# AbnerVictor/OOD-GAN-inversion

Hardware: AMD Instinct MI355X
Metric: 1024² face inversions/sec (100 W+ steps) (higher is better)
Workload: dtype f16-split (hi+lo f16 operands, f32 accumulate): 3 MFMA/product in every forward conv (fp32-equivalent), 2 in the input-gradient convs (back-propagated gradient rounded to f16 before each contraction, weights keep hi+lo); dL/dW+ vs the float64 reference 1.4e-5..3.6e-5 ('f16s': 1.3e-5..2.6e-5, the ref

## Files before the change

ood-gan-inversion_amd/csrc/conv_f16s_t2big.hip:

```cpp
#include "conv_common.hpp"
#include "sform.hpp"
#include <cstdint>
#include <cstdlib>
#include <type_traits>

using namespace oodgan;

typedef _Float16 half8 __attribute__((ext_vector_type(8)));
typedef __attribute__((address_space(3))) void lds_void;

namespace {

constexpr int TB_R = 9, TB_C = 33;
constexpr int TB_XSLOTS = TB_R * TB_C * 4;
constexpr int TB_XPIECES = (TB_XSLOTS + 63) / 64;
constexpr int TB_XBYTES = TB_XPIECES * 1024;
constexpr int TB_WPIECES = 36;
constexpr int TB_PIECES = TB_XPIECES + TB_WPIECES;
constexpr int TB_NPW = 7;
constexpr int TB_STAGE = (TB_PIECES + 1) * 1024;
constexpr int TB_CST = 2 * TB_STAGE;
constexpr int TB_SMEM = TB_CST + 64 * 4;

struct T2Big {
    oodgan_conv_args a;
    const uint4* xs;
    SDims xd;
    const float* w_unscale;
    int Hn, Wn, Hout, Wout, tiles_x, tiles_y, mblocks, Mp;
    long out_plane;
    int etiles;
    int etotal, eblocks;
};

constexpr int TE_RECS = 257;

template <bool EDGE>
__device__ __forceinline__ void t2big_body(const T2Big& p, const uint4* __restrict__ wpk16, unsigned char* smem, int w) {
    const oodgan_conv_args& a = p.a;
    const int tid = threadIdx.x, lane = tid & 63;
    const int wave = __builtin_amdgcn_readfirstlane(tid >> 6);
    const int l31 = lane & 31, half = lane >> 5;

    const int mblk = w % p.mblocks;
    w /= p.mblocks;
    const int ntile = EDGE ? p.etiles : p.tiles_x * p.tiles_y;
    const int tile = w % ntile, b = w / ntile;
    const int r0 = (tile / p.tiles_x) * 8, c0 = (tile % p.tiles_x) * 32, m0 = mblk * 64;
    const int e0 = tile * 256;
    const int M = a.M, H = p.Hn, W = p.Wn;

    unsigned off[TB_NPW];
#pragma unroll
    for (int i = 0; i < TB_NPW; ++i) {
        int pc = wave + 8 * i;
        if (pc >= TB_PIECES) pc = TB_PIECES - 1;
        if (pc < TB_XPIECES && EDGE) {
            const int P = pc * 64 + lane, rec = P >> 2, e = e0 - 1 + rec;
            int prow = 0, pcol = 0;
            if (rec < TE_RECS && e <= W) { prow = H; pcol = e + 1; }
            else if (rec < TE_RECS && e <= W + H) { prow = e - W; pcol = W; }
            off[i] = (unsigned)((((long)prow * p.xd.Wp + pcol) * 4 + (P & 3)) * 16);
        } else if (pc < TB_XPIECES) {
            int P = pc * 64 + lane;
            if (P >= TB_XSLOTS) P = TB_XSLOTS - 1;
            const int row = P / (TB_C * 4), q = P % (TB_C * 4);
            const int c = q >> 2, s = ((q & 3) - ((c >> 2) & 3)) & 3;
            off[i] = (unsigned)((((long)(r0 + row) * p.xd.Wp + (c0 + c)) * 4 + s) * 16);
        } else {
            const int u = (pc - TB_XPIECES) * 64 + lane;
            off[i] = (unsigned)((((long)(u >> 6) * p.Mp) + m0 + (u & 63)) * 16);
        }
    }
    const unsigned char* xb = reinterpret_cast<const unsigned char*>(p.xs) + (long)b * p.xd.KC * p.xd.plane * 16;
    const long xplane_bytes = p.xd.plane * 16;
    const unsigned char* wb = reinterpret_cast<const unsigned char*>(wpk16);
    const long wchunk_bytes = (long)36 * p.Mp * 16;
    const int nchunk = (a.K + 15) / 16;

    auto dma_piece = [&](int t, int buf, int i) {
        int pc = wave + 8 * i;
        if (pc >= TB_PIECES) pc = TB_PIECES - 1;
        const unsigned char* src = (pc < TB_XPIECES ? xb + (long)t * xplane_bytes : wb + (long)t * wchunk_bytes) + off[i];
        __builtin_amdgcn_global_load_lds((const __attribute__((address_space(1))) void*)src, (lds_void*)(smem + buf * TB_STAGE + pc * 1024), 16, 0, 0);
    };
    auto dma_stage = [&](int t, int buf) {
#pragma unroll
        for (int i = 0; i < TB_NPW; ++i) dma_piece(t, buf, i);
    };

    f32x16 acc[2][4];
#pragma unroll
    for (int mt = 0; mt < 2; ++mt)
#pragma unroll
        for (int ph = 0; ph < 4; ++ph)
#pragma unroll
            for (int r = 0; r < 16; ++r) acc[mt][ph][r] = 0.f;

    unsigned lrd[2][2][2];
#pragma unroll
    for (int da = 0; da < 2; ++da)
#pragma unroll
        for (int db = 0; db < 2; ++db)
#pragma unroll
            for (int lo = 0; lo < 2; ++lo) {
                if (EDGE) {
                    const int el = 32 * wave + l31, e = e0 + el;
                    int rec = TE_RECS;
                    if (e <= W) { if (da == 1) rec = el + 1 - db; }
                    else if (e <= W + H) { if (db == 1) rec = el + 1 - da; }
                    lrd[da][db][lo] = rec * 64 + (((half + 2 * lo) & 3) << 4);
                    continue;
                }
                const int c = l31 + 1 - db;
                lrd[da][db][lo] = ((wave + 1 - da) * TB_C + c) * 64 + (((half + 2 * lo + ((c >> 2) & 3)) & 3) << 4);
            }
    const unsigned lwf = (half * 64 + l31) * 16;

    struct AFrag { half8 ah[2], al[2]; };
    auto load_a = [&](AFrag& f, const unsigned char* lw, auto tp_c) {
        constexpr int tp = decltype(tp_c)::value;
#pragma unroll
        for (int mt = 0; mt < 2; ++mt) {
            f.ah[mt] = *reinterpret_cast<const half8*>(lw + (((tp * 2 + 0) * 2) * 64 + mt * 32) * 16);
            f.al[mt] = *reinterpret_cast<const half8*>(lw + (((tp * 2 + 1) * 2) * 64 + mt * 32) * 16);
        }
    };
    half8 bh[2][2], bl[2][2];
    auto mfma_tap = [&](const AFrag& f, auto tp_c) {
        constexpr int tp = decltype(tp_c)::value;
        constexpr int ky = tp / 3, kx = tp % 3, ph = (ky & 1) * 2 + (kx & 1), da = ky >> 1, db = kx >> 1;
#pragma unroll
        for (int mt = 0; mt < 2; ++mt) acc[mt][ph] = __builtin_amdgcn_mfma_f32_32x32x16_f16(f.ah[mt], bh[da][db], acc[mt][ph], 0, 0, 0);
#pragma unroll
        for (int mt = 0; mt < 2; ++mt) acc[mt][ph] = __builtin_amdgcn_mfma_f32_32x32x16_f16(f.ah[mt], bl[da][db], acc[mt][ph], 0, 0, 0);
#pragma unroll
        for (int mt = 0; mt < 2; ++mt) acc[mt][ph] = __builtin_amdgcn_mfma_f32_32x32x16_f16(f.al[mt], bh[da][db], acc[mt][ph], 0, 0, 0);
    };
#define TB_IC(n) std::integral_constant<int, n>{}
#define TB_SB() __builtin_amdgcn_sched_barrier(0)
    float cst_o = 0.f;
    if (tid < 64 && m0 + tid < M) cst_o = a.out_scale ? a.out_scale[(long)b * a.out_scale_stride + m0 + tid] : 1.f;
    dma_stage(0, 0);
    if (tid < 64) {
        reinterpret_cast<float*>(smem + TB_CST)[tid] = cst_o;
        __builtin_amdgcn_s_waitcnt(0xC07F);
    }
    for (int t = 0; t < nchunk; ++t) {
        __builtin_amdgcn_s_waitcnt(0x0F70);
        __builtin_amdgcn_s_barrier();
        const bool pf = t + 1 < nchunk;
        const int nb = (t + 1) & 1;
#define TB_DMA(i) if (pf) dma_piece(t + 1, nb, (i));
        const unsigned char* lx = smem + (t & 1) * TB_STAGE;
        const unsigned char* lw = lx + TB_XBYTES + lwf;
#pragma unroll
        for (int da = 0; da < 2; ++da)
#pragma unroll
            for (int db = 0; db < 2; ++db) {
                bh[da][db] = *reinterpret_cast<const half8*>(lx + lrd[da][db][0]);
                bl[da][db] = *reinterpret_cast<const half8*>(lx + lrd[da][db][1]);
            }
        AFrag f0, f1;
        load_a(f0, lw, TB_IC(0));
        TB_SB();
        load_a(f1, lw, TB_IC(1)); TB_DMA(0) TB_SB(); mfma_tap(f0, TB_IC(0)); TB_SB();
        load_a(f0, lw, TB_IC(3)); TB_DMA(1) TB_SB(); mfma_tap(f1, TB_IC(1)); TB_SB();
        load_a(f1, lw, TB_IC(4)); TB_DMA(2) TB_SB(); mfma_tap(f0, TB_IC(3)); TB_SB();
        load_a(f0, lw, TB_IC(2)); TB_DMA(3) TB_SB(); mfma_tap(f1, TB_IC(4)); TB_SB();
        load_a(f1, lw, TB_IC(7)); TB_DMA(4) TB_SB(); mfma_tap(f0, TB_IC(2)); TB_SB();
        load_a(f0, lw, TB_IC(5)); TB_DMA(5) TB_SB(); mfma_tap(f1, TB_IC(7)); TB_SB();
        load_a(f1, lw, TB_IC(6)); TB_DMA(6) TB_SB(); mfma_tap(f0, TB_IC(5)); TB_SB();
        load_a(f0, lw, TB_IC(8)); TB_SB(); mfma_tap(f1, TB_IC(6)); TB_SB();
        mfma_tap(f0, TB_IC(8));
#undef TB_DMA
    }
#undef TB_IC
#undef TB_SB

    const float us = (p.w_unscale ? p.w_unscale[0] : 1.f) * (a.in_mul2 ? a.in_mul2[0] : 1.f);
    float* yb = a.y + (long)b * M * p.out_plane;
    const float* cst = reinterpret_cast<const float*>(smem + TB_CST);
    if constexpr (EDGE) {
        const int e = e0 + 32 * wave + l31;
        if (e > W + H) return;
        const bool rowt = e <= W;
        const int ie = e - W - 1;
#pragma unroll
        for (int mt = 0; mt < 2; ++mt)
#pragma unroll
            for (int r = 0; r < 16; ++r) {
                const int m = m0 + mt * 32 + (r & 3) + 8 * (r >> 2) + 4 * half;
                if (m >= M) continue;
                const float sc = cst[m - m0] * us;
                float* zp = yb + (long)m * p.out_plane;
                if (rowt) {
                    float* q = zp + (long)(2 * H) * a.out_pitch + 2 * e;
                    q[0] = acc[mt][0][r] * sc;
                    if (e < W) q[1] = acc[mt][1][r] * sc;
                } else {
                    zp[(long)(2 * ie) * a.out_pitch + 2 * W] = acc[mt][0][r] * sc;
                    zp[(long)(2 * ie + 1) * a.out_pitch + 2 * W] = acc[mt][2][r] * sc;
                }
            }
        return;
    }
    const int ip = r0 + wave, jp = c0 + l31;
    const int zx = 2 * jp;
    if (ip >= H || jp >= W) return;
#pragma unroll
    for (int mt = 0; mt < 2; ++mt)
#pragma unroll
        for (int r = 0; r < 16; ++r) {
            const int m = m0 + mt * 32 + (r & 3) + 8 * (r >> 2) + 4 * half;
            if (m >= M) continue;
            const float sc = cst[m - m0] * us;
#pragma unroll
            for (int py = 0; py < 2; ++py) {
                const int zy = 2 * ip + py;
                if (zy >= p.Hout) continue;
                *reinterpret_cast<float2*>(yb + (long)m * p.out_plane + (long)zy * a.out_pitch + zx) =
                    make_float2(acc[mt][py * 2 + 0][r] * sc, acc[mt][py * 2 + 1][r] * sc);
            }
        }
}


__global__ __launch_bounds__(512) void conv_f16s_t2big_kernel(const T2Big p, const uint4* __restrict__ wpk16) {
    extern __shared__ __attribute__((aligned(16))) unsigned char smem[];
    const int bid = blockIdx.x;
    if (bid < p.eblocks) {
        if (bid < p.etotal) t2big_body<true>(p, wpk16, smem, bid);
        return;
    }
    t2big_body<false>(p, wpk16, smem, xcd_remap(bid - p.eblocks, gridDim.x - p.eblocks));
}

}

namespace oodgan {

bool t2_big_eligible(const oodgan_conv_args& a) {
    if (!(a.mode == OODGAN_CONV_T2 && a.x_sform && a.M >= 64 && a.y != nullptr && a.in_scale == nullptr && a.in_shift == nullptr &&
          a.dotx == nullptr && a.noise == nullptr && a.bias == nullptr && a.act == OODGAN_ACT_NONE && a.ys == nullptr))
        return false;
    const long items = (long)((a.Hin + 7) / 8) * ((a.Win + 31) / 32) * a.B * ((a.M + 63) / 64);
    return items >= tunable(OODGAN_TUN_T2_BIG_MIN_ITEMS);
}

int launch_t2_big(const oodgan_conv_args& a_in, const void* wpk16, const float* unscale, hipStream_t st) {
    T2Big p;
    p.a = a_in;
    oodgan_conv_args& a = p.a;
    p.Hn = a.Hin; p.Wn = a.Win; p.Hout = 2 * a.Hin + 1; p.Wout = 2 * a.Win + 1;
    if (a.out_pitch == 0) a.out_pitch = p.Wout + 1;
    OODGAN_REQUIRE((a.out_pitch & 1) == 0 && a.out_pitch >= p.Wout + 1, "conv3x3 T2: out_pitch must be even and > 2W+1 (got %d)", a.out_pitch);
    p.out_plane = (long)p.Hout * a.out_pitch;
    p.xs = reinterpret_cast<const uint4*>(a.x);
    p.xd = sform_dims(a.K, a.Hin, a.Win);
    p.w_unscale = unscale;
    p.tiles_y = (p.Hn + 7) / 8;
    p.tiles_x = (p.Wn + 31) / 32;
    p.Mp = (a.M + 63) / 64 * 64;
    p.mblocks = (a.M + 63) / 64;
    OODGAN_REQUIRE(p.xd.plane * 16 < (1L << 32), "conv3x3 T2 big: input plane too large");
    p.etiles = (a.Hin + a.Win + 1 + 255) / 256;
    const long total = (long)p.tiles_x * p.tiles_y * a.B * p.mblocks, etotal = (long)p.etiles * a.B * p.mblocks;
    OODGAN_REQUIRE(total > 0 && total < (1L << 31), "conv3x3: grid too large");
    static bool once = ((void)hipFuncSetAttribute(reinterpret_cast<const void*>(&conv_f16s_t2big_kernel), hipFuncAttributeMaxDynamicSharedMemorySize, TB_SMEM), true);
    (void)once;
    static_assert(TE_RECS * 4 + 4 <= TB_XPIECES * 64, "edge records + the zero record fit the x region");
    p.etotal = (int)etotal;
    p.eblocks = (int)((etotal + 7) / 8 * 8);
    OODGAN_REQUIRE(total + p.eblocks < (1L << 31), "conv3x3: grid too large");
    hipLaunchKernelGGL(conv_f16s_t2big_kernel, dim3((unsigned)(total + p.eblocks)), dim3(512), TB_SMEM, st, p, reinterpret_cast<const uint4*>(wpk16));
    return check_launch("conv3x3_f16s_t2big");
}

}
```

Measured before the change: 7.881.

## Specialize edge blocks of the T2 transposed conv to load only needed taps

The edge (last row/column) blocks of the stride-2 transposed 3x3 conv now fetch only the x records and the three weight taps that contribute to each edge phase. Previously they ran the full nine-tap loop against mostly zero records. Row and column edges are split into separate tiles aligned to 256, and only live waves issue MFMAs. A three-buffer ring with two-deep prefetch and per-count waitcnts replaces the double buffer. The cost is more complex edge indexing, though edge blocks are a small part of the total grid.

New measurement: 7.931, median of 4. No clear change (+0.6%).

```diff
diff --git a/ood-gan-inversion_amd/csrc/conv_f16s_t2big.hip b/ood-gan-inversion_amd/csrc/conv_f16s_t2big.hip
--- a/ood-gan-inversion_amd/csrc/conv_f16s_t2big.hip
+++ b/ood-gan-inversion_amd/csrc/conv_f16s_t2big.hip
@@ -29,11 +29,18 @@
     const float* w_unscale;
     int Hn, Wn, Hout, Wout, tiles_x, tiles_y, mblocks, Mp;
     long out_plane;
+    int ecol0;
     int etiles;
     int etotal, eblocks;
 };
 
 constexpr int TE_RECS = 257;
+constexpr int TE_XPIECES = (TE_RECS * 4 + 63) / 64;
+constexpr int TE_XBYTES = TE_XPIECES * 1024;
+constexpr int TE_NPW = 4;
+constexpr int TE_STAGE = (TE_XPIECES + 12) * 1024;
+constexpr int TE_NBUF = 3;
+static_assert(TE_NBUF * TE_STAGE <= TB_CST, "the edge ring stays below the out-scale slots");
 
 template <bool EDGE>
 __device__ __forceinline__ void t2big_body(const T2Big& p, const uint4* __restrict__ wpk16, unsigned char* smem, int w) {
@@ -50,18 +57,35 @@
     const int e0 = tile * 256;
     const int M = a.M, H = p.Hn, W = p.Wn;
 
+    const int R = p.ecol0;
+    const bool e_roww = e0 < R;
+    const int e_npos = min(256, (e_roww ? W + 1 : R + H) - e0);
+    const int e_xp = ((e_npos + 31) / 32 * 32 + 1 + 15) >> 4;
+    const int e_npieces = e_xp + 12, e_npw = (e_npieces + 7) >> 3;
+    const bool e_live = 32 * wave < e_npos;
+
     unsigned off[TB_NPW];
 #pragma unroll
     for (int i = 0; i < TB_NPW; ++i) {
         int pc = wave + 8 * i;
+        if (EDGE) {
+            if (i >= TE_NPW) break;
+            if (pc >= e_npieces) pc = e_npieces - 1;
+            if (pc < e_xp) {
+                const int P = pc * 64 + lane, rec = P >> 2, e = e0 - 1 + rec;
+                int prow = 0, pcol = 0;
+                if (rec < TE_RECS && e <= W) { prow = H; pcol = e + 1; }
+                else if (rec < TE_RECS && e >= R && e < R + H) { prow = e - R + 1; pcol = W; }
+                off[i] = (unsigned)((((long)prow * p.xd.Wp + pcol) * 4 + (P & 3)) * 16);
+            } else {
+                const int j = pc - e_xp, slot = j >> 2;
+                const int tap = slot == 0 ? 8 : e_roww ? 5 + slot : 3 * slot - 1;
+                off[i] = (unsigned)((((long)(tap * 4 + (j & 3)) * p.Mp) + m0 + lane) * 16);
+            }
+            continue;
+        }
         if (pc >= TB_PIECES) pc = TB_PIECES - 1;
-        if (pc < TB_XPIECES && EDGE) {
-            const int P = pc * 64 + lane, rec = P >> 2, e = e0 - 1 + rec;
-            int prow = 0, pcol = 0;
-            if (rec < TE_RECS && e <= W) { prow = H; pcol = e + 1; }
-            else if (rec < TE_RECS && e <= W + H) { prow = e - W; pcol = W; }
-            off[i] = (unsigned)((((long)prow * p.xd.Wp + pcol) * 4 + (P & 3)) * 16);
-        } else if (pc < TB_XPIECES) {
+        if (pc < TB_XPIECES) {
             int P = pc * 64 + lane;
             if (P >= TB_XSLOTS) P = TB_XSLOTS - 1;
             const int row = P / (TB_C * 4), q = P % (TB_C * 4);
@@ -88,6 +112,17 @@
 #pragma unroll
         for (int i = 0; i < TB_NPW; ++i) dma_piece(t, buf, i);
     };
+    auto dma_edge_stage = [&](int t, int buf) {
+#pragma unroll
+        for (int i = 0; i < TE_NPW; ++i) {
+            if (i >= e_npw) break;
+            int pc = wave + 8 * i;
+            if (pc >= e_npieces) pc = e_npieces - 1;
+            const unsigned char* src = (pc < e_xp ? xb + (long)t * xplane_bytes : wb + (long)t * wchunk_bytes) + off[i];
+            const int lp = pc < e_xp ? pc : pc - e_xp + TE_XPIECES;
+            __builtin_amdgcn_global_load_lds((const __attribute__((address_space(1))) void*)src, (lds_void*)(smem + buf * TE_STAGE + lp * 1024), 16, 0, 0);
+        }
+    };
 
     f32x16 acc[2][4];
 #pragma unroll
@@ -105,11 +140,7 @@
 #pragma unroll
             for (int lo = 0; lo < 2; ++lo) {
                 if (EDGE) {
-                    const int el = 32 * wave + l31, e = e0 + el;
-                    int rec = TE_RECS;
-                    if (e <= W) { if (da == 1) rec = el + 1 - db; }
-                    else if (e <= W + H) { if (db == 1) rec = el + 1 - da; }
-                    lrd[da][db][lo] = rec * 64 + (((half + 2 * lo) & 3) << 4);
+                    lrd[da][db][lo] = (32 * wave + l31 + 1 - db) * 64 + (((half + 2 * lo) & 3) << 4);
                     continue;
                 }
                 const int c = l31 + 1 - db;
@@ -127,26 +158,66 @@
         }
     };
     half8 bh[2][2], bl[2][2];
+    auto mfma_ph = [&](const AFrag& f, const half8& xh, const half8& xl, auto ph_c) {
+        constexpr int ph = decltype(ph_c)::value;
+#pragma unroll
+        for (int mt = 0; mt < 2; ++mt) acc[mt][ph] = __builtin_amdgcn_mfma_f32_32x32x16_f16(f.ah[mt], xh, acc[mt][ph], 0, 0, 0);
+#pragma unroll
+        for (int mt = 0; mt < 2; ++mt) acc[mt][ph] = __builtin_amdgcn_mfma_f32_32x32x16_f16(f.ah[mt], xl, acc[mt][ph], 0, 0, 0);
+#pragma unroll
+        for (int mt = 0; mt < 2; ++mt) acc[mt][ph] = __builtin_amdgcn_mfma_f32_32x32x16_f16(f.al[mt], xh, acc[mt][ph], 0, 0, 0);
+    };
     auto mfma_tap = [&](const AFrag& f, auto tp_c) {
         constexpr int tp = decltype(tp_c)::value;
         constexpr int ky = tp / 3, kx = tp % 3, ph = (ky & 1) * 2 + (kx & 1), da = ky >> 1, db = kx >> 1;
-#pragma unroll
-        for (int mt = 0; mt < 2; ++mt) acc[mt][ph] = __builtin_amdgcn_mfma_f32_32x32x16_f16(f.ah[mt], bh[da][db], acc[mt][ph], 0, 0, 0);
-#pragma unroll
-        for (int mt = 0; mt < 2; ++mt) acc[mt][ph] = __builtin_amdgcn_mfma_f32_32x32x16_f16(f.ah[mt], bl[da][db], acc[mt][ph], 0, 0, 0);
-#pragma unroll
-        for (int mt = 0; mt < 2; ++mt) acc[mt][ph] = __builtin_amdgcn_mfma_f32_32x32x16_f16(f.al[mt], bh[da][db], acc[mt][ph], 0, 0, 0);
+        mfma_ph(f, bh[da][db], bl[da][db], std::integral_constant<int, ph>{});
     };
 #define TB_IC(n) std::integral_constant<int, n>{}
 #define TB_SB() __builtin_amdgcn_sched_barrier(0)
     float cst_o = 0.f;
     if (tid < 64 && m0 + tid < M) cst_o = a.out_scale ? a.out_scale[(long)b * a.out_scale_stride + m0 + tid] : 1.f;
-    dma_stage(0, 0);
+    if constexpr (EDGE) {
+        dma_edge_stage(0, 0);
+        if (nchunk > 1) dma_edge_stage(1, 1);
+    } else {
+        dma_stage(0, 0);
+    }
     if (tid < 64) {
         reinterpret_cast<float*>(smem + TB_CST)[tid] = cst_o;
         __builtin_amdgcn_s_waitcnt(0xC07F);
     }
-    for (int t = 0; t < nchunk; ++t) {
+    auto edge_loop = [&](auto ph0_c, auto ph1_c) {
+        constexpr int ph0 = decltype(ph0_c)::value, ph1 = decltype(ph1_c)::value;
+        const unsigned char* lw0 = smem + TE_XBYTES + lwf + (e_roww ? 2 : 1) * 4096;
+        const unsigned char* lw1 = smem + TE_XBYTES + lwf + (e_roww ? 1 : 2) * 4096;
+        const unsigned char* lw2 = smem + TE_XBYTES + lwf;
+        for (int t = 0, buf = 0; t < nchunk; ++t, buf = buf + 1 == TE_NBUF ? 0 : buf + 1) {
+            if (t + 1 == nchunk) __builtin_amdgcn_s_waitcnt(0x0F70);
+            else if (e_npw == 4) __builtin_amdgcn_s_waitcnt(0x0F74);
+            else if (e_npw == 3) __builtin_amdgcn_s_waitcnt(0x0F73);
+            else __builtin_amdgcn_s_waitcnt(0x0F72);
+            __builtin_amdgcn_s_barrier();
+            if (t + 2 < nchunk) dma_edge_stage(t + 2, buf == 0 ? TE_NBUF - 1 : buf - 1);
+            if constexpr (ph0 >= 0) {
+                const unsigned char* lx = smem + buf * TE_STAGE;
+                const half8 ch = *reinterpret_cast<const half8*>(lx + lrd[1][0][0]), cl = *reinterpret_cast<const half8*>(lx + lrd[1][0][1]);
+                const half8 qh = *reinterpret_cast<const half8*>(lx + lrd[1][1][0]), ql = *reinterpret_cast<const half8*>(lx + lrd[1][1][1]);
+                AFrag f0, f1, f2;
+                load_a(f0, lw0 + buf * TE_STAGE, TB_IC(0));
+                load_a(f1, lw1 + buf * TE_STAGE, TB_IC(0));
+                load_a(f2, lw2 + buf * TE_STAGE, TB_IC(0));
+                mfma_ph(f0, ch, cl, ph0_c);
+                mfma_ph(f1, ch, cl, ph1_c);
+                mfma_ph(f2, qh, ql, TB_IC(0));
+            }
+        }
+    };
+    if constexpr (EDGE) {
+        if (!e_live) edge_loop(TB_IC(-1), TB_IC(-1));
+        else if (e_roww) edge_loop(TB_IC(1), TB_IC(0));
+        else edge_loop(TB_IC(0), TB_IC(2));
+    }
+    for (int t = 0; !EDGE && t < nchunk; ++t) {
         __builtin_amdgcn_s_waitcnt(0x0F70);
         __builtin_amdgcn_s_barrier();
         const bool pf = t + 1 < nchunk;
@@ -183,9 +254,9 @@
     const float* cst = reinterpret_cast<const float*>(smem + TB_CST);
     if constexpr (EDGE) {
         const int e = e0 + 32 * wave + l31;
-        if (e > W + H) return;
-        const bool rowt = e <= W;
-        const int ie = e - W - 1;
+        const bool rowt = e_roww;
+        const int ie = e - R;
+        if (rowt ? e > W : ie >= H) return;
 #pragma unroll
         for (int mt = 0; mt < 2; ++mt)
 #pragma unroll
@@ -264,12 +335,12 @@
     p.Mp = (a.M + 63) / 64 * 64;
     p.mblocks = (a.M + 63) / 64;
     OODGAN_REQUIRE(p.xd.plane * 16 < (1L << 32), "conv3x3 T2 big: input plane too large");
-    p.etiles = (a.Hin + a.Win + 1 + 255) / 256;
+    p.ecol0 = (a.Win + 1 + 255) / 256 * 256;
+    p.etiles = (p.ecol0 + a.Hin + 255) / 256;
     const long total = (long)p.tiles_x * p.tiles_y * a.B * p.mblocks, etotal = (long)p.etiles * a.B * p.mblocks;
     OODGAN_REQUIRE(total > 0 && total < (1L << 31), "conv3x3: grid too large");
     static bool once = ((void)hipFuncSetAttribute(reinterpret_cast<const void*>(&conv_f16s_t2big_kernel), hipFuncAttributeMaxDynamicSharedMemorySize, TB_SMEM), true);
     (void)once;
-    static_assert(TE_RECS * 4 + 4 <= TB_XPIECES * 64, "edge records + the zero record fit the x region");
     p.etotal = (int)etotal;
     p.eblocks = (int)((etotal + 7) / 8 * 8);
     OODGAN_REQUIRE(total + p.eblocks < (1L << 31), "conv3x3: grid too large");
```
